# rongzhao-zhang/EfficientQ

Measured on AMD Instinct MI355X. Metric: ptq_calibration_throughput, higher is better.
Workload: dtype i8xi8->i32 (exact) for the Gram systems and per-iteration loss convs of the layers with quantised input, f32/f64 elsewhere

## Files before the change

efficientq_amd/_lib.py:

```python
from __future__ import annotations

import ctypes as C
import os

import torch

_HERE = os.path.dirname(os.path.abspath(__file__))
LIB_PATH = os.path.join(_HERE, "libeffq_hip.so")

EFFQ_OK = 0
_ERR_NAMES = {1: "EFFQ_ERR_ARG", 2: "EFFQ_ERR_HIP", 3: "EFFQ_ERR_WORKSPACE", 4: "EFFQ_ERR_NO_DEVICE",
              5: "EFFQ_ERR_NOT_CONVERGED"}


class EffqError(RuntimeError):
    pass


class Geom(C.Structure):
    _fields_ = [(n, C.c_int32) for n in
                ("N", "C1", "C2", "D", "H", "W", "KD", "KH", "KW", "SD", "SH", "SW", "PD", "PH", "PW")]

    def out_dims(self):
        return ((self.D + 2 * self.PD - self.KD) // self.SD + 1,
# ... 80 lines not shown
    "effq_fp_check": (_I, [_P, _P, _P]),
    "effq_fp_channels_max_row": (_I, []),
    "effq_fixed_point_channels": (_I, [_P, _P, _P, _I, _I, _I, _D, _I, _P, _P, _P, _P]),
    "effq_fixed_point_channels_proj": (_I, [_P, _P, _P, _I, _I, _I, _D, _I, _P, _P, _P, _P, _F, _P, _P, _P, _I, _I, _D,
                                            _D, _P]),
    "effq_gram_packed_elems": (_SZ, [_I, _I]),
    "effq_gram_pack": (_I, [_P, _P, _I, _I, _P, _P]),
    "effq_gram_unpack": (_I, [_P, _I, _I, _P, _P, _P]),
    "effq_act_quant_backward": (_I, [_P, _P, _I, _P, _P, _P, _SZ, _P, _P]),
    "effq_att_classes_ws_bytes": (_SZ, []),
    "effq_att_classes": (_I, [_P, _LL, _P, _P, _P, C.POINTER(C.c_int32), _P, _P]),
    "effq_prof_enable": (_I, [_I]),
    "effq_prof_count": (_I, []),
    "effq_prof_read": (_I, [_I, C.POINTER(ProfRecord)]),
    "effq_admm_num_inverses": (_I, [_D, _D, _I, _I]),
    "effq_admm_run": (_I, [C.POINTER(AdmmRunArgs)]),
    "effq_admm_select_best": (_I, [_P, _I, _P, _P, _SZ, _SZ, _P, _P, _P, _P]),
    "effq_gram_ws_bytes": (_SZ, [_GP, _I]),
    "effq_gram_accum": (_I, [_P, _P, _P, _GP, _I, _P, _P, _I, _P, _SZ, _P]),
    "effq_gram_plan_query": (_I, [_GP, _I, _IP, _IP, _IP, _IP, _LLP, _IP, _IP]),
    "effq_gram_i8_supported": (_I, [_GP, _I]),
    "effq_gram_i8_ws_bytes": (_SZ, [_GP, _I]),
    "effq_gram_accum_i8": (_I, [_P, _P, _GP, _I, _P, _I, _P, _P, _P, _I, _LL, _P, _P, _I, _P, _SZ, _P]),
    "effq_gram_accum_i8_unw": (_I, [_P, _P, _GP, _I, _P, _I, _P, _P, _P, _I, _LL, _P, _P, _I, _P, _P, _P, _SZ, _P]),
    "effq_gram_i8_plan_query": (_I, [_GP, _I, _LL, _IP, _IP, _IP, _IP, _IP, _IP]),
    "effq_gram_i8_group_query": (_I, [_GP, _I, _LL, _IP, _IP, _IP, _IP]),
    "effq_gram_i8_set_group": (_I, [_I, _I]),
    "effq_upsample_trilinear": (_I, [_P, _I, _I, _I, _I, _I, _I, _I, _I, _P, _P]),
    "effq_gram_f64_supported": (_I, [_GP, _I]),
    "effq_gram_f64_ws_bytes": (_SZ, [_GP, _I]),
    "effq_gram_f64": (_I, [_P, _P, _GP, _I, _P, _P, _P, _SZ, _P]),
    "effq_gram_f64_plan_query": (_I, [_GP, _I, _IP, _IP, _IP, _IP]),
    "effq_gram_f64_pipelined": (_I, [_P, _P, _GP, _I]),
    "effq_gram_loss_ws_bytes": (_SZ, [_I]),
    "effq_gram_loss": (_I, [_P, _P, _P, _P, _P, _I, _I, _I, _P, _P, _SZ, _P]),
    "effq_packed_bytes": (_SZ, [_SZ, _I]),
    "effq_pack_levels": (_I, [_P, _SZ, _I, _P, _P]),
    "effq_unpack_levels": (_I, [_P, _SZ, _I, _P, _P]),
    "effq_ainv_ld": (_I, [_I]),
    "effq_fp_bracket_export_words": (_SZ, []),
    "effq_fp_bracket_export": (_I, [_P, _SZ, _P, _P, _SZ, _P]),
    "effq_fp_bracket_rebase": (_I, [_P, _P, _SZ, _P]),
    "effq_fp_bracket_import": (_I, [_P, _SZ, _P, _I, _SZ, _P, _P, _SZ, _P]),
    "effq_admm_uses_traj": (_I, [_SZ, _I]),
    "effq_gram_loss_i8_supported": (_I, [_I, _I, _I, _I]),
    "effq_gram_loss_i8_num_planes": (_I, [C.c_longlong]),
    "effq_gram_loss_i8_planes_bytes": (_SZ, [_I, _I, _I]),
    "effq_gram_loss_i8_prepare": (_I, [_P, _I, _I, _P, _I, _I, _P, _P, _P]),
    "effq_gram_loss_i8_ws_bytes": (_SZ, []),
    "effq_gram_loss_i8": (_I, [_P, _I, _P, _P, _P, _P, _P, _P, _P, _I, _I, _I, _I, _I, _I, _P, _P, _SZ, _P]),
    "effq_spd_inverse_ws_bytes": (_SZ, [_I]),
    "effq_spd_inverse": (_I, [_P, _I, _I, _D, _D, _P, _P, _SZ, _P]),
    "effq_spd_inverse_plan": (_I, [_I, _IP, _IP, _IP]),
    "effq_prox_plan_query": (_I, [_I, _I, _IP, _IP, _IP, _IP]),
    "effq_prox_ws_bytes": (_SZ, [_I, _I]),
    "effq_prox_solve": (_I, [_P, _P, _P, _P, _P, _P, _I, _I, _I, _D, _D, _P, _P, _P, _SZ, _P]),
    "effq_prox_solve_shifted": (_I, [_P, _P, _P, _P, _P, _P, _I, _I, _I, _D, _D, _D, _I, _P, _P, _P, _SZ, _P]),
    "effq_admm_presum": (_I, [_P, _P, _P, _SZ, _P]),
    "effq_admm_project_dual": (_I, [_P, _P, _P, _I, _P, _P, _F, _P, _SZ, _P]),
    "effq_conv_plan_query": (_I, [_GP, _I, _IP, _IP, _IP, _IP, _IP, _IP, _IP, _IP, _LLP]),
    "effq_conv_i8_plan_query": (_I, [_GP, _I, _IP, _IP, _IP, _IP]),
    "effq_conv_i8s_plan_query": (_I, [_GP, _I, _I, _IP, _IP, _IP, _IP, _IP, _IP, _IP]),
    "effq_conv_i8_supported": (_I, [_GP, _I, _I]),
    "effq_conv_i8s_supported": (_I, [_GP, _I, _I]),
    "effq_conv_i8s_ws_bytes": (_SZ, [_GP, _I, _I]),
    "conv3d_calib_step_i8s": (_I, [_P, _P, _P, _P, _GP, _P, _I, _P, _I, _I, _P, _P, _SZ, _P]),
    "effq_conv_i8_ws_bytes": (_SZ, [_GP]),
    "conv3d_calib_step_i8": (_I, [_P, _P, _P, _P, _GP, _P, _I, _P, _I, _P, _P, _SZ, _P]),
    "effq_conv_i8_out_supported": (_I, [_GP, _I, _I]),
    "conv3d_quant_forward_i8": (_I, [_P, _P, _P, _P, _P, _GP, _P, _I, _P, _I, _P, _P, _P, _SZ, _P]),
    "effq_conv_ws_bytes": (_SZ, [_GP]),
    "conv3d_quant_calib_step": (_I, [_P, _P, _P, _P, _P, _GP, _P, _I, _P, _P, _P, _SZ, _P]),
    "effq_adam_step": (_I, [_P, _P, _P, _P, _D, _D, _D, _D, _I, _SZ, _P]),
    "effq_window_gather": (_I, [_P, _I, _I, _I, _I, _I, _I, _I, _I, _I, _I, _I, _I, _I, _I, _P, _P]),
    "effq_window_put": (_I, [_P, _I, _I, _I, _I, _I, _I, _I, _P, _P]),
    "effq_window_stitch": (_I, [_P, _I, _I, _I, _I, _I, _I, _I, _I, _I, _I, _I, _P, _P, _P, _I, _P, _P]),
    "effq_seg_tallies": (_I, [_P, _P, _I, _LL, _I, _I, _F, _P, _P, _SZ, _P]),
    "effq_seg_sweep": (_I, [_P, _P, _I, _LL, _I, _I, _F, _P, _P]),
    "effq_seg_sweep_edges": (_I, [_I, _F, _P]),
    "effq_seg_sweep_plan": (_I, [_I, _LL, _I, _IP, _IP]),
    "effq_seg_labels": (_I, [_P, _I, _I, _LL, _I, _I, _F, _I, _P, _P]),
    "effq_seg_labels_source": (_I, [_P, _I, _P, _P, _P, _P, _P, _I, _I, _F, _P, _P]),
    "effq_seg_probs_source": (_I, [_P, _I, _P, _P, _P, _P, _P, _I, _P, _P, _P]),
    "effq_seg_agreement": (_I, [_P, _P, _I, _LL, _I, _I, _F, _P, _P, _P, _P, _P, _SZ, _P]),
    "effq_cc_ws_bytes": (_SZ, [_I, _I, _I, _I]),
    "effq_cc_label": (_I, [_P, _I, _I, _I, _I, _I, _P, _P, _P, _SZ, _P]),
    "effq_seg_lesions": (_I, [_P, _P, _I, _I, _I, _I, _I, _I, _F, _I, _P, _P, _SZ, _P]),
    "effq_cc_table_ws_bytes": (_SZ, [_I, _I, _I, _I, _I]),
    "effq_cc_table": (_I, [_P, _I, _I, _I, _I, _I, _I, _P, _P, _P, _SZ, _P]),
    "effq_seg_lesion_table": (_I, [_P, _P, _I, _I, _I, _I, _I, _I, _F, _I, _I, _P, _P, _P, _P, _SZ, _P]),
    "effq_label_clean_ws_bytes": (_SZ, [_I, _I, _I]),
    "effq_label_clean": (_I, [_P, _I, _I, _I, _I, _I, _P, _P, _P, _P, _P, _SZ, _P]),
    "effq_label_tallies_ws_bytes": (_SZ, []),
    "effq_label_tallies": (_I, [_P, _P, _I, _I, _LL, _P, _P, _P, _SZ, _P]),
    "effq_surf_ws_bytes": (_SZ, [_I, _I, _I, _I]),
    "effq_edt_sq": (_I, [_P, _I, _I, _I, _I, _P, _P, _SZ, _P]),
    "effq_seg_surface": (_I, [_P, _P, _I, _I, _I, _I, _I, _I, _F, _P, _P, _P, _SZ, _P]),
    "effq_surf_mm_ws_bytes": (_SZ, [_I, _I, _I, _I]),
    "effq_edt_sq_mm": (_I, [_P, _I, _I, _I, _I, _F, _F, _F, _P, _P, _SZ, _P]),
    "effq_seg_surface_mm": (_I, [_P, _P, _I, _I, _I, _I, _I, _I, _F, _F, _F, _F, _P, _P, _P, _P, _SZ, _P]),
    "effq_prep_window": (_I, [_P, _SZ, _F, _F, _P]),
    "effq_prep_resample": (_I, [_P, _I, _I, _I, _I, _D, _D, _D, _I, _P, _I, _I, _I, _P]),
    "effq_prep_bbox_moments": (_I, [_P, _I, _I, _I, _I, _I, _P, _P, _P, _P, _SZ, _P]),
    "effq_prep_sqdev": (_I, [_P, _I, _LL, _I, _P, _P, _P, _SZ, _P]),
    "effq_prep_standardise_crop": (_I, [_P, _I, _I, _I, _I, _I, _P, _P, _P, _P, _P, _P]),
    "effq_prep_crop_u8": (_I, [_P, _I, _I, _I, _I, _P, _P, _P, _P]),
# ... 47 lines not shown
```

efficientq_amd/csrc/solve.hip:

```cpp
#include <cstdlib>
#include <vector>
#include "common.h"
#include "internal.h"

namespace effq {

typedef float f32x16 __attribute__((ext_vector_type(16)));
typedef double f64x4 __attribute__((ext_vector_type(4)));
typedef float f32x4 __attribute__((ext_vector_type(4)));

static inline int round_up(int v, int m) { return (v + m - 1) / m * m; }

constexpr int NBK = 64;
constexpr int LDA_S = 66;
constexpr int LDB_S = 80;

__global__ __launch_bounds__(256) void k_build_a64(const float* __restrict__ A0, int n, int npad, int has_bias,
                                                   double rho, double eta, double* __restrict__ A64) {
  const size_t tot = (size_t)npad * npad;
  const size_t stride = (size_t)gridDim.x * blockDim.x;
  for (size_t e = (size_t)blockIdx.x * blockDim.x + threadIdx.x; e < tot; e += stride) {
    const int i = (int)(e / npad), j = (int)(e % npad);
    double v = 0.0;
    if (i < n && j < n) {
// ... 87 lines not shown
                                                  double* __restrict__ XT) {
  extern __shared__ __attribute__((aligned(16))) double sm[];
  double* As = sm;
  double* Bs = sm + NBK * LDA_S;
  const int kblk = kb / NBK;
  const int t = blockIdx.x;
  const int tid = threadIdx.x, lane = tid & 63, wid = tid >> 6;
  const int wr = wid >> 1, wc = wid & 1;
  if (t == kblk) {
    for (int e = tid; e < NBK * NBK; e += 256) A[(size_t)(kb + (e >> 6)) * npad + kb + (e & 63)] = Dinv[e];
    return;
  }
  const bool upper = t < kblk;
  const double sgn = upper ? -1.0 : 1.0;
  for (int e = tid; e < NBK * NBK; e += 256) {
    const int r = e >> 6, c = e & 63;
    const double v = upper ? A[(size_t)(t * NBK + r) * npad + kb + c] : A[(size_t)(kb + r) * npad + (size_t)t * NBK + c];
    if (upper) {
      As[r * LDA_S + c] = v;
    } else {
      As[c * LDA_S + r] = v;
    }
  }
  load_tile(Bs, LDB_S, Dinv, NBK);
  lds_barrier();
  for (int e = tid; e < NBK * NBK; e += 256) {
    const int kk = e >> 6, r = e & 63;
    XT[(size_t)kk * npad + (size_t)t * NBK + r] = sgn * As[r * LDA_S + kk];
  }
  f64x4 acc[2][2];
#pragma unroll
  for (int mi = 0; mi < 2; ++mi)
#pragma unroll
    for (int ni = 0; ni < 2; ++ni)
#pragma unroll
      for (int r = 0; r < 4; ++r) acc[mi][ni][r] = 0.0;
  tile_mma64(As, Bs, acc);
  const int lr = lane & 15, lk = lane >> 4;
#pragma unroll
  for (int mi = 0; mi < 2; ++mi)
#pragma unroll
    for (int ni = 0; ni < 2; ++ni)
#pragma unroll
      for (int r = 0; r < 4; ++r) {
        const int row = wr * 32 + mi * 16 + lk + 4 * r;
        const int col = wc * 32 + ni * 16 + lr;
        const double z = acc[mi][ni][r];
        NZ[(size_t)(t * NBK + row) * NBK + col] = -z;
        if (upper)
          A[(size_t)(t * NBK + row) * npad + kb + col] = -z;
        else
          A[(size_t)(kb + col) * npad + (size_t)t * NBK + row] = z;
      }
}

__global__ __launch_bounds__(256) void k_gj_trail_sym(double* __restrict__ A, int npad, int kb,
                                                      const double* __restrict__ NZ, const double* __restrict__ XT,
                                                      double* __restrict__ Dinv_next) {
  __shared__ __attribute__((aligned(16))) double As[NBK * LDA_S];
  __shared__ double fcol[2][NBK + 1];
  const int kblk = kb / NBK, nblk = npad / NBK;
  const int kn = kblk + 1;
  const bool ahead = Dinv_next != nullptr && kn < nblk;
  const int tid = threadIdx.x, lane = tid & 63, wid = tid >> 6;
  const int wr = wid >> 1, wc = wid & 1;
  const int lr = lane & 15, lk = lane >> 4;
  if (blockIdx.y == 0) {
    if (blockIdx.x != 0 || !ahead) return;
    for (int e = tid; e < NBK * NBK; e += 256) {
      const int r = e >> 6, c = e & 63;
      As[r * LDA_S + c] = NZ[(size_t)(kn * NBK + r) * NBK + c];
    }
    lds_barrier();
    const double* Cb = A + (size_t)(kn * NBK + wr * 32) * npad + (size_t)kn * NBK + wc * 32;
    const double* Rb = XT + (size_t)kn * NBK + wc * 32;
    f64x4 acc[2][2];
#pragma unroll
    for (int mi = 0; mi < 2; ++mi)
#pragma unroll
      for (int ni = 0; ni < 2; ++ni)
#pragma unroll
        for (int r = 0; r < 4; ++r) acc[mi][ni][r] = Cb[(size_t)(mi * 16 + lk + 4 * r) * npad + ni * 16 + lr];
#pragma unroll 4
    for (int ks = 0; ks < NBK / 4; ++ks) {
      double a[2], b[2];
#pragma unroll
      for (int mi = 0; mi < 2; ++mi) a[mi] = As[(wr * 32 + mi * 16 + lr) * LDA_S + ks * 4 + lk];
#pragma unroll
      for (int ni = 0; ni < 2; ++ni) b[ni] = Rb[(size_t)(ks * 4 + lk) * npad + ni * 16 + lr];
#pragma unroll
      for (int mi = 0; mi < 2; ++mi)
#pragma unroll
        for (int ni = 0; ni < 2; ++ni) acc[mi][ni] = __builtin_amdgcn_mfma_f64_16x16x4f64(a[mi], b[ni], acc[mi][ni], 0, 0, 0);
    }
    lds_barrier();
#pragma unroll
    for (int mi = 0; mi < 2; ++mi)
#pragma unroll
      for (int ni = 0; ni < 2; ++ni)
#pragma unroll
        for (int r = 0; r < 4; ++r)
          As[(wr * 32 + mi * 16 + lk + 4 * r) * LDA_S + wc * 32 + ni * 16 + lr] = acc[mi][ni][r];
    lds_barrier();
    constexpr int CPW = NBK / 4;
    double reg[CPW];
#pragma unroll
    for (int j = 0; j < CPW; ++j) reg[j] = As[lane * LDA_S + wid * CPW + j];
    gj_invert_regs<CPW>(reg, fcol, lane, wid);
#pragma unroll
    for (int j = 0; j < CPW; ++j) Dinv_next[lane * NBK + wid * CPW + j] = reg[j];
    return;
  }
  const int ib = (int)blockIdx.y - 1;
  if (ib == kblk) return;
  if ((int)(blockIdx.x * GJ_CT + GJ_CT - 1) < ib) return;
  for (int e = tid; e < NBK * NBK; e += 256) {
    const int r = e >> 6, c = e & 63;
    As[r * LDA_S + c] = NZ[(size_t)(ib * NBK + r) * NBK + c];
  }
  lds_barrier();
  auto live = [&](int t) -> bool {
    const int jb = blockIdx.x * GJ_CT + t;
    return t < GJ_CT && jb < nblk && jb != kblk && jb >= ib && !(ahead && ib == kn && jb == kn);
  };
  auto fetch = [&](int t, f64x4 (&c)[2][2]) {
    const int jb = blockIdx.x * GJ_CT + t;
    const double* Cb = A + (size_t)(ib * NBK + wr * 32) * npad + (size_t)jb * NBK + wc * 32;
#pragma unroll
    for (int mi = 0; mi < 2; ++mi)
#pragma unroll
      for (int ni = 0; ni < 2; ++ni)
#pragma unroll
        for (int r = 0; r < 4; ++r) c[mi][ni][r] = Cb[(size_t)(mi * 16 + lk + 4 * r) * npad + ni * 16 + lr];
  };
  f64x4 nxt[2][2];
  int t = 0;
  while (t < GJ_CT && !live(t)) ++t;
  if (t < GJ_CT) fetch(t, nxt);
  while (t < GJ_CT) {
    const int jb = blockIdx.x * GJ_CT + t;
    f64x4 acc[2][2];
#pragma unroll
    for (int mi = 0; mi < 2; ++mi)
#pragma unroll
      for (int ni = 0; ni < 2; ++ni) acc[mi][ni] = nxt[mi][ni];
    int tn = t + 1;
    while (tn < GJ_CT && !live(tn)) ++tn;
    if (tn < GJ_CT) fetch(tn, nxt);
    double* Cb = A + (size_t)(ib * NBK + wr * 32) * npad + (size_t)jb * NBK + wc * 32;
    const double* Rb = XT + (size_t)jb * NBK + wc * 32;
#pragma unroll 4
    for (int ks = 0; ks < NBK / 4; ++ks) {
      double a[2], b[2];
#pragma unroll
      for (int mi = 0; mi < 2; ++mi) a[mi] = As[(wr * 32 + mi * 16 + lr) * LDA_S + ks * 4 + lk];
#pragma unroll
      for (int ni = 0; ni < 2; ++ni) b[ni] = Rb[(size_t)(ks * 4 + lk) * npad + ni * 16 + lr];
#pragma unroll
      for (int mi = 0; mi < 2; ++mi)
#pragma unroll
        for (int ni = 0; ni < 2; ++ni) acc[mi][ni] = __builtin_amdgcn_mfma_f64_16x16x4f64(a[mi], b[ni], acc[mi][ni], 0, 0, 0);
    }
#pragma unroll
    for (int mi = 0; mi < 2; ++mi)
#pragma unroll
      for (int ni = 0; ni < 2; ++ni)
#pragma unroll
        for (int r = 0; r < 4; ++r) Cb[(size_t)(mi * 16 + lk + 4 * r) * npad + ni * 16 + lr] = acc[mi][ni][r];
    t = tn;
  }
}

__global__ __launch_bounds__(256) void k_a64_to_f32(const double* __restrict__ A64, int n, int npad,
                                                    float* __restrict__ Ainv, int lda) {
  const size_t tot = (size_t)n * lda;
  const size_t stride = (size_t)gridDim.x * blockDim.x;
  for (size_t e = (size_t)blockIdx.x * blockDim.x + threadIdx.x; e < tot; e += stride) {
    const int i = (int)(e / lda), j = (int)(e % lda);
    const int a = (i < j) ? i : j, b = (i < j) ? j : i;
    Ainv[e] = (j < n) ? (float)A64[(size_t)a * npad + b] : 0.0f;
  }
}

constexpr int WB = 4, WK = WB * NBK;
constexpr int BG_T = 128, BG_KC = 16, BG_LD = 144;
typedef double f64x2 __attribute__((ext_vector_type(2)));

struct GjBig {
  const double* Cin;
  size_t ldin;
  double* Cout;
  size_t ldout;
  int orow, ocol;
  const double* NZT;
  const double* XTW;
  size_t ldx;
  int kdim;
  int nblk;
  int i0m, j0m;
  int skip_lo, skip_hi;
  int la_lo, la_hi;
};

__global__ __launch_bounds__(256, 2) void k_gj_big(const GjBig p) {
  __shared__ __attribute__((aligned(16))) double As[2][BG_KC * BG_LD];
  __shared__ __attribute__((aligned(16))) double Bs[2][BG_KC * BG_LD];
  const int I = p.i0m + (int)blockIdx.y, J = p.j0m + (int)blockIdx.x;
  if (J < I) return;
  auto blk_live = [&](int bi, int bj) -> bool {
    if (bi > bj || bj >= p.nblk) return false;
    if ((bi >= p.skip_lo && bi < p.skip_hi) || (bj >= p.skip_lo && bj < p.skip_hi)) return false;
    if (bi >= p.la_lo && bi < p.la_hi && bj >= p.la_lo && bj < p.la_hi) return false;
    return true;
  };
  if (!(blk_live(2 * I, 2 * J) || blk_live(2 * I, 2 * J + 1) || blk_live(2 * I + 1, 2 * J) || blk_live(2 * I + 1, 2 * J + 1)))
    return;
  const int tid = threadIdx.x, lane = tid & 63, wid = tid >> 6;
  const int wr = wid >> 1, wc = wid & 1;
  const int lr = lane & 15, lk = lane >> 4;
  const int bi = 2 * I + wr, bj = 2 * J + wc;
  const bool live = blk_live(bi, bj);
  f64x4 acc[4][4];
  if (live) {
// ... 653 lines not shown
    int s5 = (256 + tiles5 / 2) / tiles5;
    if (s5 > nkt5 / 16) s5 = nkt5 / 16;
    if (s5 < 1) s5 = 1;
    p.nsplit = s5;
    return p;
  }
  if (p.c2p >= 256) { p.variant = 0; p.gx = (n + 63) / 64; p.gy = p.c2p / 256; }
  else if (p.c2p == 128) { p.variant = 1; p.gx = (n + 63) / 64; p.gy = 1; }
  else if (p.c2p == 64) { p.variant = 2; p.gx = (n + 63) / 64; p.gy = 1; }
  else { p.variant = 3; p.gx = (n + 127) / 128; p.gy = 1; }
  const int tiles = p.gx * p.gy, nkt = p.ldb / PBK;
  int s = (440 + tiles - 1) / tiles;
  if (s > nkt / 6) s = nkt / 6;
  if (s > 16) s = 16;
  if (s < 1) s = 1;
  if (p.variant == 0) {
    const int smax = s > 1 ? 16 : 1;
    double best = -1.0;
    for (int c = 1; c <= smax && c <= nkt / 6; ++c) {
      const int wgs = tiles * c, rounds = (wgs + 767) / 768;
      const double score = (double)wgs / (768.0 * rounds) - 0.01 * c;
      if (score > best) { best = score; s = c; }
    }
  }
  p.nsplit = s;
  return p;
}

}

using namespace effq;

extern "C" {

static size_t gj64_aux_doubles(size_t npad) { return 2 * (size_t)NBK * npad + 2 * NBK * NBK; }

constexpr int GJ_WIDE_MIN_BLOCKS = 100;
static bool gj_takes_wide(int nblk) { return nblk >= GJ_WIDE_MIN_BLOCKS; }
static int gj_wide_pivot(int nblk) { return (nblk >= 100) ? effq::WB : 2; }

size_t effq_spd_inverse_ws_bytes(int n) {
  if (n <= 0) return 0;
  const size_t npad = (size_t)round_up(n, NBK);
  size_t d = npad * npad + gj64_aux_doubles(npad);
  if (gj_takes_wide((int)(npad / NBK))) {
    const size_t ldx = (size_t)round_up((int)npad, BG_T);
    d = npad * npad + 2 * (size_t)WK * ldx + (size_t)WK * WK + gj64_aux_doubles(WK);
  }
  return d * sizeof(double) + 256;
}

int effq_ainv_ld(int n) { return n > 0 ? round_up(n, 32) : 0; }

static int gj64_sweep(double* A64, int npad, double* aux, hipStream_t st) {
  const int nblk = npad / NBK;
  double* XT = aux;
  double* NZ = XT + (size_t)NBK * npad;
  double* Dinv = NZ + (size_t)NBK * npad;
  const size_t lds = (size_t)(NBK * LDA_S + NBK * LDB_S) * sizeof(double);
  for (int k = 0; k < nblk; ++k) {
    const int kb = k * NBK;
    double* Dk = Dinv + (size_t)(k & 1) * NBK * NBK;
    double* Dn = Dinv + (size_t)((k + 1) & 1) * NBK * NBK;
    if (k == 0) hipLaunchKernelGGL(k_gj_diag, dim3(1), dim3(GJD_T), 0, st, A64, npad, kb, Dk);
    hipLaunchKernelGGL(k_gj_panel, dim3(nblk), dim3(256), lds, st, A64, npad, kb, Dk, NZ, XT);
    if (nblk > 1)
      hipLaunchKernelGGL(k_gj_trail_sym, dim3((nblk + GJ_CT - 1) / GJ_CT, nblk + 1), dim3(256), 0, st, A64, npad, kb, NZ,
                         XT, Dn);
    EFFQ_LAUNCH_CHECK();
  }
  return EFFQ_OK;
}

struct GjWideCtx {
  int dev;
  hipStream_t caller, helper;
  hipEvent_t e1, e2;
};
static thread_local std::vector<GjWideCtx> g_gj_ctx;

static int gj_wide_ctx(hipStream_t caller, GjWideCtx** out) {
  int dev = 0;
  EFFQ_HIP(hipGetDevice(&dev));
  for (GjWideCtx& c : g_gj_ctx)
    if (c.dev == dev && c.caller == caller) {
      *out = &c;
      return EFFQ_OK;
    }
  GjWideCtx c;
  c.dev = dev;
  c.caller = caller;
  int prio = 0;
  if (hipStreamGetPriority(caller, &prio) != hipSuccess) prio = 0;
  EFFQ_HIP(hipStreamCreateWithPriority(&c.helper, hipStreamNonBlocking, prio));
  EFFQ_HIP(hipEventCreateWithFlags(&c.e1, hipEventDisableTiming));
  EFFQ_HIP(hipEventCreateWithFlags(&c.e2, hipEventDisableTiming));
  g_gj_ctx.push_back(c);
  *out = &g_gj_ctx.back();
  return EFFQ_OK;
}

static int gj_wide_sweep(double* A64, int npad, double* aux, hipStream_t st) {
  const int nblk = npad / NBK;
  const int WB = gj_wide_pivot(nblk);
  const size_t ldx = (size_t)round_up(npad, BG_T);
  double* NZT = aux;
  double* XTW = NZT + (size_t)WK * ldx;
  double* Dw = XTW + (size_t)WK * ldx;
  double* aux64 = Dw + (size_t)WK * WK;
  const int nK = (nblk + WB - 1) / WB, nm = (nblk + 1) / 2;
  GjWideCtx* ctx = nullptr;
  if (nK > 1) {
    const int rc = gj_wide_ctx(st, &ctx);
    if (rc != EFFQ_OK) return rc;
  }
  hipStream_t s2 = ctx ? ctx->helper : st;
  const size_t lds = (size_t)(NBK * LDA_S + NBK * LDB_S) * sizeof(double);
  const size_t pf_lds = (size_t)(2 * NBK * PF_LD + 2 * (NBK + 1)) * sizeof(double);
  auto pivot_block = [&](int k0, int mk, int kdim, hipStream_t s) -> int {
// ... 33 lines not shown
    }
    hipLaunchKernelGGL(k_gj_wback_w, dim3(nblk, m), dim3(256), 0, s2, A64, npad, kb0, m, Dw, NZT, ldx);
    EFFQ_LAUNCH_CHECK();
    if (mn > 0) {
      const int rc = pivot_block(kn0, mn, m * NBK, s2);
      if (rc != EFFQ_OK) return rc;
    }
    if (nblk > m) {
      GjBig g;
      memset(&g, 0, sizeof(g));
      g.Cin = A64; g.ldin = (size_t)npad;
      g.Cout = A64; g.ldout = (size_t)npad; g.orow = 0; g.ocol = 0;
      g.NZT = NZT; g.XTW = XTW; g.ldx = ldx; g.kdim = m * NBK; g.nblk = nblk;
      g.i0m = 0; g.j0m = 0;
      g.skip_lo = kb0; g.skip_hi = kb0 + m;
      g.la_lo = mn > 0 ? kn0 : -1; g.la_hi = mn > 0 ? kn0 + mn : -1;
      hipLaunchKernelGGL(k_gj_big, dim3(nm, nm), dim3(256), 0, st, g);
      EFFQ_LAUNCH_CHECK();
    }
    if (ctx) {
      EFFQ_HIP(hipEventRecord(ctx->e2, s2));
      EFFQ_HIP(hipStreamWaitEvent(st, ctx->e2, 0));
    }
  }
  return EFFQ_OK;
}

int effq_spd_inverse_prepare(void* stream) {
  GjWideCtx* ctx = nullptr;
  return gj_wide_ctx(as_stream(stream), &ctx);
}

int effq_spd_inverse(const float* A0, int n, int has_bias, double rho, double eta, float* Ainv, void* ws,
                     size_t ws_bytes, void* stream) {
  EFFQ_CHECK_ARG(A0 && Ainv && ws && n > 0);
  EFFQ_CHECK_ARG(eta > 0.0 && rho >= 0.0);
  if (ws_bytes < effq_spd_inverse_ws_bytes(n)) {
    set_error("spd_inverse: workspace %zu < required %zu", ws_bytes, effq_spd_inverse_ws_bytes(n));
    return EFFQ_ERR_WORKSPACE;
  }
  const int npad = round_up(n, NBK);
  double* A64 = reinterpret_cast<double*>(ws);
  double* aux = A64 + (size_t)npad * npad;
  hipStream_t st = as_stream(stream);
  {
    size_t nb = ((size_t)npad * npad + 255) / 256;
    if (nb > 8192) nb = 8192;
    hipLaunchKernelGGL(k_build_a64, dim3((unsigned)nb), dim3(256), 0, st, A0, n, npad, has_bias, rho, eta, A64);
    EFFQ_LAUNCH_CHECK();
  }
  const size_t lds = (size_t)(NBK * LDA_S + NBK * LDB_S) * sizeof(double);
  EFFQ_HIP(raise_lds_limit<k_gj_panel>(lds));
  EFFQ_HIP(raise_lds_limit<k_gj_panel_w>(lds));
  EFFQ_HIP(raise_lds_limit<k_gj_pivot_fused>((2 * NBK * PF_LD + 2 * (NBK + 1)) * sizeof(double)));
  const int rc = gj_takes_wide(npad / NBK) ? gj_wide_sweep(A64, npad, aux, st) : gj64_sweep(A64, npad, aux, st);
  if (rc != EFFQ_OK) return rc;
  {
    const int lda = effq_ainv_ld(n);
    size_t nb = ((size_t)n * lda + 255) / 256;
    if (nb > 8192) nb = 8192;
    hipLaunchKernelGGL(k_a64_to_f32, dim3((unsigned)nb), dim3(256), 0, st, A64, n, npad, Ainv, lda);
    EFFQ_LAUNCH_CHECK();
  }
  return EFFQ_OK;
}

int effq_spd_inverse_plan(int n, int* wide, int* nblk, int* pivot_blocks) {
  EFFQ_CHECK_ARG(n > 0 && wide && nblk && pivot_blocks);
  const int nb = round_up(n, NBK) / NBK;
  *wide = gj_takes_wide(nb) ? 1 : 0;
  *nblk = nb;
  *pivot_blocks = *wide ? (nb + gj_wide_pivot(nb) - 1) / gj_wide_pivot(nb) : nb;
  return EFFQ_OK;
}

int effq_prox_plan_query(int c2, int n, int* variant, int* gx, int* gy, int* nsplit) {
  EFFQ_CHECK_ARG(c2 > 0 && n > 0 && variant && gx && gy && nsplit);
  const ProxPlan p = prox_plan(c2, n);
  *variant = p.variant;
  *gx = p.gx;
  *gy = p.gy;
  *nsplit = p.nsplit;
  return EFFQ_OK;
}

size_t effq_prox_ws_bytes(int c2, int n) {
  if (c2 <= 0 || n <= 0) return 0;
  const ProxPlan p = prox_plan(c2, n);
  return ((size_t)p.c2p + (p.nsplit > 1 ? (size_t)p.nsplit * c2 : 0)) * p.ldb * sizeof(float) + 256;
}

static int prox_solve_impl(const float* B0, const float* Ainv, const float* W0, const float* b0, const float* G,
                           const float* dual, int c2, int n, int has_bias, double rho, double eta, double shift,
                           int nterms, float* wstar, float* bstar, void* ws, size_t ws_bytes, void* stream,
                           bool prebuilt = false, const float** part_out = nullptr, int* nsplit_out = nullptr,
                           int* ldp_out = nullptr) {
  EFFQ_CHECK_ARG(B0 && Ainv && W0 && G && dual && wstar && ws && c2 > 0 && n > 0 && nterms >= 1);
  EFFQ_CHECK_ARG(!has_bias || (b0 != nullptr && bstar != nullptr));
  if (ws_bytes < effq_prox_ws_bytes(c2, n)) {
    set_error("prox_solve: workspace %zu < required %zu", ws_bytes, effq_prox_ws_bytes(c2, n));
    return EFFQ_ERR_WORKSPACE;
  }
  const ProxPlan pl = prox_plan(c2, n);
  const int c2p = pl.c2p, ldb = pl.ldb;
  const int lda = effq_ainv_ld(n);
  float* Bm = reinterpret_cast<float*>(ws);
  float* part = Bm + (size_t)c2p * ldb;
  hipStream_t st = as_stream(stream);
  for (int term = 0; term < nterms; ++term) {
    if (!(prebuilt && term == 0)) {
      const int nw = n - (has_bias ? 1 : 0);
      if ((nw % 4) == 0) {
        const unsigned bx = (unsigned)((ldb / 4 + 255) / 256);
        hipLaunchKernelGGL(k_build_b4, dim3(bx, (unsigned)c2p), dim3(256), 0, st, B0, W0, b0, G, dual, c2, n,
                           has_bias ? 1 : 0, (float)rho, (float)eta, Bm, ldb, (term > 0) ? wstar : nullptr, (float)shift);
      } else {
        size_t nb = ((size_t)c2p * ldb + 255) / 256;
        if (nb > 4096) nb = 4096;
        hipLaunchKernelGGL(k_build_b, dim3((unsigned)nb), dim3(256), 0, st, B0, W0, b0, G, dual, c2, n, has_bias ? 1 : 0,
                           (float)rho, (float)eta, Bm, ldb, c2p, (term > 0) ? wstar : nullptr, (float)shift);
      }
      EFFQ_LAUNCH_CHECK();
    }
    const dim3 grid(pl.gx, pl.gy, pl.nsplit);
#define EFFQ_PROX_LAUNCH(MT, WM, WN, NTN)                                                                              \
  hipLaunchKernelGGL((k_prox_gemm<MT, WM, WN, NTN>), grid, dim3(256), 0, st, Bm, ldb, Ainv, lda, n, c2, has_bias ? 1 : 0, \
                     wstar, bstar, part, ldb)
// ... 79 lines not shown
```

efficientq_amd/hip_ops.py:

```python
from __future__ import annotations

import ctypes as C
import math
from typing import Optional, Tuple

import torch

from . import _lib
from ._lib import Geom, check

ADMM_TOL = 1e-5
FP_BRACKET_MIN = 1 << 18
DP_GATHER_AFTER = 4
DP_GATHER_MAX_BYTES = 128 << 20


def _ptr(t: Optional[torch.Tensor]):
    return None if t is None else C.c_void_p(t.data_ptr())


def to_ndhwc(x: torch.Tensor) -> torch.Tensor:
    return x.permute(0, 2, 3, 4, 1).contiguous()


# ... 534 lines not shown
        check(self.lib.effq_gram_loss_i8(_ptr(planes), int(planes.shape[0]), _ptr(Au), _ptr(Bu), _ptr(syy), _ptr(Gq), _ptr(b),
                                         _ptr(states), _ptr(al), int(act_levels), int(w_levels), c2, n, int(has_b), count,
                                         _ptr(hist), _ptr(ws), ws.numel(), self.stream), "effq_gram_loss_i8")
        return hist

    def gram_reduce(self, A0: torch.Tensor, B0: torch.Tensor, reducer):
        n, c2 = int(A0.shape[0]), int(B0.shape[0])
        buf = torch.empty(self.lib.effq_gram_packed_elems(n, c2), dtype=torch.float32, device=self.device)
        check(self.lib.effq_gram_pack(_ptr(A0), _ptr(B0), n, c2, _ptr(buf), self.stream), "effq_gram_pack")
        reducer(buf)
        check(self.lib.effq_gram_unpack(_ptr(buf), n, c2, _ptr(A0), _ptr(B0), self.stream), "effq_gram_unpack")
        return A0, B0

    @staticmethod
    def storage_bits(levels: int) -> int:
        for b in (1, 2, 4, 8):
            if levels <= (1 << b):
                return b
        raise _lib.EffqError(f"{levels} levels do not fit 8 bits")

    def pack_levels(self, idx: torch.Tensor, bits: int) -> torch.Tensor:
        if idx.dtype != torch.uint8 or not idx.is_contiguous():
            raise _lib.EffqError("pack_levels wants contiguous uint8 level ids")
        nb = self.lib.effq_packed_bytes(idx.numel(), int(bits))
        if idx.numel() and nb == 0:
            raise _lib.EffqError(f"unsupported field width {bits}")
        out = torch.empty(int(nb), dtype=torch.uint8, device=idx.device)
        check(self.lib.effq_pack_levels(_ptr(idx), idx.numel(), int(bits), _ptr(out), self.stream), "effq_pack_levels")
        return out

    def unpack_levels(self, packed: torch.Tensor, n: int, bits: int) -> torch.Tensor:
        if packed.dtype != torch.uint8 or packed.numel() != self.lib.effq_packed_bytes(int(n), int(bits)):
            raise _lib.EffqError("unpack_levels: buffer does not match n and the field width")
        out = torch.empty(int(n), dtype=torch.uint8, device=packed.device)
        check(self.lib.effq_unpack_levels(_ptr(packed.contiguous()), int(n), int(bits), _ptr(out), self.stream),
              "effq_unpack_levels")
        return out

    def spd_inverse(self, A0: torch.Tensor, has_bias: bool, rho: float, eta: float,
                    out: Optional[torch.Tensor] = None, ws_key: str = "inv") -> torch.Tensor:
        n = A0.shape[0]
        A0 = self._f32(A0)
        if out is None:
            out = torch.empty(n, self.lib.effq_ainv_ld(n), dtype=torch.float32, device=self.device)
        ws = self._workspace(ws_key, self.lib.effq_spd_inverse_ws_bytes(n))
        check(self.lib.effq_spd_inverse(_ptr(A0), n, int(has_bias), rho, eta, _ptr(out), _ptr(ws), ws.numel(),
                                        self.stream), "effq_spd_inverse")
        return out

    def spd_inverse_plan(self, n: int) -> dict:
        wide, nblk, piv = C.c_int(), C.c_int(), C.c_int()
        check(self.lib.effq_spd_inverse_plan(int(n), C.byref(wide), C.byref(nblk), C.byref(piv)), "effq_spd_inverse_plan")
        return dict(wide=bool(wide.value), nblk=nblk.value, pivot_blocks=piv.value)

    def prox_plan(self, c2: int, n: int) -> dict:
        v, gx, gy, ns = C.c_int(), C.c_int(), C.c_int(), C.c_int()
        check(self.lib.effq_prox_plan_query(int(c2), int(n), C.byref(v), C.byref(gx), C.byref(gy), C.byref(ns)),
              "effq_prox_plan_query")
        return dict(variant=v.value, gx=gx.value, gy=gy.value, nsplit=ns.value)

    def prox_solve(self, B0, Ainv, W0, b0, G, dual, rho: float, eta: float, wstar, bstar):
        c2, n = B0.shape
        ws = self._workspace("prox", self.lib.effq_prox_ws_bytes(c2, n))
        check(self.lib.effq_prox_solve(_ptr(B0), _ptr(Ainv), _ptr(W0), _ptr(b0), _ptr(G), _ptr(dual), c2, n,
                                       int(b0 is not None), rho, eta, _ptr(wstar), _ptr(bstar), _ptr(ws),
                                       ws.numel(), self.stream), "effq_prox_solve")

    PROX_SHIFT_TERMS = 26

    def prox_solve_shifted(self, B0, Ainv, W0, b0, G, dual, rho: float, eta: float, rho_inv: float, wstar, bstar):
        c2, n = B0.shape
        ws = self._workspace("prox", self.lib.effq_prox_ws_bytes(c2, n))
        terms = self.shift_terms(rho, eta, rho_inv)
        check(self.lib.effq_prox_solve_shifted(_ptr(B0), _ptr(Ainv), _ptr(W0), _ptr(b0), _ptr(G), _ptr(dual), c2, n,
                                               int(b0 is not None), rho, eta, rho_inv, terms, _ptr(wstar),
                                               _ptr(bstar), _ptr(ws), ws.numel(), self.stream),
              "effq_prox_solve_shifted")

    def admm_run(self, A0, B0, W0, b0, geom: Geom, y_ndhwc, *, xq=None, xidx=None, act_alpha=None, act_levels: int = 0,
                 loss_kind: int = 0, rho: float, rho_max: float, eta: float, iters: int, period: int, levels: int,
                 overlap: bool = True, loss_gram=None, residuals: bool = False, channel_wise: bool = False):
        from types import SimpleNamespace
        c2, n = (int(i) for i in B0.shape)
        has_b = b0 is not None
        W0, A0, B0 = self._f32(W0), self._f32(A0), self._f32(B0)
        b0 = self._f32(b0) if has_b else None
        xq = self._f32(xq) if xq is not None else None
        nw = W0.numel()
        y = self._f32(y_ndhwc)
        planes = None
        if loss_gram is not None and len(loss_gram) == 4:
            loss_kind = 5
            planes = loss_gram[3]
            loss_gram = loss_gram[:3]
        elif loss_gram is not None:
            loss_kind = 4
        if channel_wise and loss_kind not in (0, 4):
            raise _lib.EffqError(f"admm_run: channel mode takes loss kinds 0 and 4, not {loss_kind}")
        _check_shapes(geom, xq if loss_kind in (0, 4, 5) else xidx, W0, b0, y)
        if tuple(A0.shape) != (n, n) or nw != c2 * (n - int(has_b)):
            raise _lib.EffqError("admm_run: A0/B0/W0 shapes do not match")
        n_inv = self.lib.effq_admm_num_inverses(float(rho), float(rho_max), int(iters), int(period))
        if n_inv < 1:
            raise _lib.EffqError("admm_run: bad rho schedule")
        dev, f32 = self.device, torch.float32
        ld = self.lib.effq_ainv_ld(n)
# ... 917 lines not shown
```

include/effq_hip.h:

```cpp
#ifndef EFFQ_HIP_H
#define EFFQ_HIP_H

#include <stddef.h>
#include <stdint.h>

#ifdef __cplusplus
extern "C" {
#endif

enum {
  EFFQ_OK = 0,
  EFFQ_ERR_ARG = 1,
  EFFQ_ERR_HIP = 2,
  EFFQ_ERR_WORKSPACE = 3,
  EFFQ_ERR_NO_DEVICE = 4,
  EFFQ_ERR_NOT_CONVERGED = 5
};

typedef struct effq_geom {
  int32_t N, C1, C2;
  int32_t D, H, W;
  int32_t KD, KH, KW;
  int32_t SD, SH, SW;
  int32_t PD, PH, PW;
// ... 86 lines not shown
                    int has_bias, float* A0, float* B0, int accumulate, void* ws, size_t ws_bytes,
                    void* stream);
int effq_gram_plan_query(const effq_geom* g, int has_bias, int* vec, int* nb, int* npairs, int* nsplit,
                         long long* vox_per_split, int* fold, int* finish_blocks);

int effq_gram_i8_supported(const effq_geom* g, int act_levels);
size_t effq_gram_i8_ws_bytes(const effq_geom* g, int ncls);
int effq_gram_accum_i8(const uint8_t* xidx_ndhwc, const float* y_ndhwc, const effq_geom* g, int has_bias,
                       const float* act_alpha_dev, int act_levels, const int32_t* vox_list,
                       const int32_t* chunk_cls, const float* cls_w_dev, int ncls, long long n_list,
                       float* A0, float* B0, int accumulate, void* ws, size_t ws_bytes, void* stream);
int effq_gram_accum_i8_unw(const uint8_t* xidx_ndhwc, const float* y_ndhwc, const effq_geom* g, int has_bias,
                           const float* act_alpha_dev, int act_levels, const int32_t* vox_list, const int32_t* chunk_cls,
                           const float* cls_w_dev, int ncls, long long n_list, float* A0, float* B0, int accumulate,
                           double* Au, double* Bu, void* ws, size_t ws_bytes, void* stream);
int effq_gram_i8_plan_query(const effq_geom* g, int ncls, long long n_list, int* nb, int* nbx, int* npairs, int* nchunks,
                            int* cps, int* nsplit);
int effq_gram_i8_group_query(const effq_geom* g, int ncls, long long n_list, int* gi, int* gj, int* ngroups, int* grid_y);
int effq_gram_i8_set_group(int gi, int gj);

int effq_gram_f64_supported(const effq_geom* g, int has_bias);
size_t effq_gram_f64_ws_bytes(const effq_geom* g, int has_bias);
int effq_gram_f64(const float* x_ndhwc, const float* y_ndhwc, const effq_geom* g, int has_bias, double* Au, double* Bu,
                  void* ws, size_t ws_bytes, void* stream);
int effq_gram_f64_plan_query(const effq_geom* g, int has_bias, int* nchunk, int* grid, int* ntiles, int* tpw);
int effq_gram_f64_pipelined(const float* x_ndhwc, const float* y_ndhwc, const effq_geom* g, int has_bias);

size_t effq_gram_loss_ws_bytes(int n);
int effq_gram_loss(const double* Au, const double* Bu, const double* syy_dev, const float* G, const float* b, int c2, int n,
                   int has_bias, double* sqerr_out, void* ws, size_t ws_bytes, void* stream);

int effq_gram_loss_i8_supported(int c2, int n, int has_bias, int w_levels);
int effq_gram_loss_i8_num_planes(long long kmax);
size_t effq_gram_loss_i8_planes_bytes(int n, int has_bias, int nplanes);
int effq_gram_loss_i8_prepare(const double* Au, int n, int has_bias, const float* act_alpha_dev, int act_levels,
                              int nplanes, int8_t* planes, int32_t* err_flag_dev, void* stream);
size_t effq_gram_loss_i8_ws_bytes(void);
int effq_gram_loss_i8(const int8_t* planes, int nplanes, const double* Au, const double* Bu, const double* syy_dev,
                      const int8_t* Gq, const float* b, const effq_fp_state* states, const float* act_alpha_dev,
                      int act_levels, int w_levels, int c2, int n, int has_bias, int count, double* hist_out, void* ws,
                      size_t ws_bytes, void* stream);


size_t effq_att_classes_ws_bytes(void);
int effq_att_classes(const float* att, long long V, int32_t* vox_list, int32_t* chunk_cls, float* cls_w_dev,
                     int32_t* info_host_out, void* ws, void* stream);

int effq_spd_inverse_prepare(void* stream);
int effq_ainv_ld(int n);
size_t effq_spd_inverse_ws_bytes(int n);
int effq_spd_inverse(const float* A0, int n, int has_bias, double rho, double eta, float* Ainv,
                     void* ws, size_t ws_bytes, void* stream);
int effq_spd_inverse_plan(int n, int* wide, int* nblk, int* pivot_blocks);

size_t effq_prox_ws_bytes(int c2, int n);
int effq_prox_solve(const float* B0, const float* Ainv, const float* W0, const float* b0, const float* G,
                    const float* dual, int c2, int n, int has_bias, double rho, double eta, float* wstar,
                    float* bstar, void* ws, size_t ws_bytes, void* stream);
int effq_prox_plan_query(int c2, int n, int* variant, int* gx, int* gy, int* nsplit);

int effq_prox_solve_shifted(const float* B0, const float* Ainv, const float* W0, const float* b0, const float* G,
                            const float* dual, int c2, int n, int has_bias, double rho, double eta,
                            double rho_inv, int nterms, float* wstar, float* bstar, void* ws, size_t ws_bytes,
                            void* stream);

int effq_admm_presum(const float* wstar, const float* dual, float* v, size_t n, void* stream);
int effq_admm_project_dual(const float* v, const float* wstar, const effq_fp_state* state_dev, int levels,
                           float* G, float* dual, float dual_div, int8_t* Gq_out, size_t n, void* stream);
size_t effq_conv_ws_bytes(const effq_geom* g);
int conv3d_quant_calib_step(const float* xq_ndhwc, const float* G, const float* bias, const float* y_fp,
                            const float* att, const effq_geom* g, const float* act_alpha_dev, int act_levels,
                            double* sqerr_out, float* out, void* ws, size_t ws_bytes, void* stream);
int effq_conv_plan_query(const effq_geom* g, int loss_only, int* kind, int* fast, int* cslab, int* nslab, int* nt,
                         int* grid_x, int* grid_y, int* ntiles, long long* lds_bytes);

int effq_conv_i8_supported(const effq_geom* g, int act_levels, int w_levels);
size_t effq_conv_i8_ws_bytes(const effq_geom* g);
int conv3d_calib_step_i8(const uint8_t* xidx_ndhwc, const int8_t* Gq, const float* bias, const float* y_fp,
                         const effq_geom* g, const float* act_alpha_dev, int act_levels,
                         const effq_fp_state* w_state_dev, int w_levels, double* sqerr_out, void* ws,
                         size_t ws_bytes, void* stream);
int effq_conv_i8_out_supported(const effq_geom* g, int act_levels, int w_levels);
int conv3d_quant_forward_i8(const uint8_t* xidx_ndhwc, const int8_t* Gq, const float* bias, const float* y_fp,
                            const float* att, const effq_geom* g, const float* act_alpha_dev, int act_levels,
                            const effq_fp_state* w_state_dev, int w_levels, double* sqerr_out, float* out, void* ws,
                            size_t ws_bytes, void* stream);
int effq_conv_i8_plan_query(const effq_geom* g, int want_out, int* kernel, int* grid_x, int* grid_y, int* ntiles);

int effq_conv_i8s_supported(const effq_geom* g, int act_levels, int w_levels);
size_t effq_conv_i8s_ws_bytes(const effq_geom* g, int act_levels, int w_levels);
int conv3d_calib_step_i8s(const uint8_t* xidx_ndhwc, const int8_t* Gq, const float* bias, const float* y_fp,
                          const effq_geom* g, const float* act_alpha_dev, int act_levels,
                          const effq_fp_state* w_state_dev, int w_levels, int prepare, double* sqerr_out,
                          void* ws, size_t ws_bytes, void* stream);
int effq_conv_i8s_plan_query(const effq_geom* g, int act_levels, int w_levels, int* nj, int* ct, int* taps, int* k,
                             int* aoff, int* wmul, int* grid);

int effq_act_quant_backward(const float* x, const float* alpha_dev, int levels, const float* gq, float* gx_out,
                            double* galpha_out, size_t n, void* ws, void* stream);
int effq_adam_step(float* p, const float* g, float* m, float* v, double lr, double b1, double b2, double eps,
                   int t, size_t n, void* stream);

typedef struct effq_admm_run_args {
  const float* A0; const float* B0; const float* W0; const float* b0;
  int32_t c2, n, has_bias, w_levels;
  int32_t iters, rho_period;
// ... 152 lines not shown
```

Measured before the change: 25.46.

## Pack four trailing-update row blocks per 1024-thread workgroup in Gauss-Jordan sweep

Adds a trailing-update kernel variant for the blocked Gauss-Jordan SPD inverse. Each 1024-thread workgroup handles four row blocks and uses 1 or 2 column tiles per strip, chosen by block count. The look-ahead diagonal inverse is computed with 16 waves instead of 4. The goal is to cut per-workgroup launch/latency overhead and raise parallelism for mid-sized matrices, at the cost of larger LDS use and a shared barrier across idle row slots. A runtime switch (default on) selects the new path.

```diff
diff --git a/efficientq_amd/_lib.py b/efficientq_amd/_lib.py
--- a/efficientq_amd/_lib.py
+++ b/efficientq_amd/_lib.py
@@ -156,6 +156,8 @@
     "effq_spd_inverse_ws_bytes": (_SZ, [_I]),
     "effq_spd_inverse": (_I, [_P, _I, _I, _D, _D, _P, _P, _SZ, _P]),
     "effq_spd_inverse_plan": (_I, [_I, _IP, _IP, _IP]),
+    "effq_spd_inverse_set_pivot": (_I, [_I]),
+    "effq_spd_inverse_pivot": (_I, []),
     "effq_prox_plan_query": (_I, [_I, _I, _IP, _IP, _IP, _IP]),
     "effq_prox_ws_bytes": (_SZ, [_I, _I]),
     "effq_prox_solve": (_I, [_P, _P, _P, _P, _P, _P, _I, _I, _I, _D, _D, _P, _P, _P, _SZ, _P]),
diff --git a/efficientq_amd/csrc/solve.hip b/efficientq_amd/csrc/solve.hip
--- a/efficientq_amd/csrc/solve.hip
+++ b/efficientq_amd/csrc/solve.hip
@@ -163,6 +163,66 @@
         else
           A[(size_t)(kb + col) * npad + (size_t)t * NBK + row] = z;
       }
+}
+
+template <int CT>
+__device__ __forceinline__ void gj_trail_strip(double* __restrict__ A, int npad, const double* __restrict__ XT,
+                                               const double* As, int ib, int strip, int kblk, int nblk, bool ahead,
+                                               int t4) {
+  const int lane = t4 & 63, wid = t4 >> 6;
+  const int wr = wid >> 1, wc = wid & 1;
+  const int lr = lane & 15, lk = lane >> 4;
+  const int kn = kblk + 1;
+  auto live = [&](int t) -> bool {
+    const int jb = strip * CT + t;
+    return t < CT && jb < nblk && jb != kblk && jb >= ib && !(ahead && ib == kn && jb == kn);
+  };
+  auto fetch = [&](int t, f64x4 (&c)[2][2]) {
+    const int jb = strip * CT + t;
+    const double* Cb = A + (size_t)(ib * NBK + wr * 32) * npad + (size_t)jb * NBK + wc * 32;
+#pragma unroll
+    for (int mi = 0; mi < 2; ++mi)
+#pragma unroll
+      for (int ni = 0; ni < 2; ++ni)
+#pragma unroll
+        for (int r = 0; r < 4; ++r) c[mi][ni][r] = Cb[(size_t)(mi * 16 + lk + 4 * r) * npad + ni * 16 + lr];
+  };
+  f64x4 nxt[2][2];
+  int t = 0;
+  while (t < CT && !live(t)) ++t;
+  if (t < CT) fetch(t, nxt);
+  while (t < CT) {
+    const int jb = strip * CT + t;
+    f64x4 acc[2][2];
+#pragma unroll
+    for (int mi = 0; mi < 2; ++mi)
+#pragma unroll
+      for (int ni = 0; ni < 2; ++ni) acc[mi][ni] = nxt[mi][ni];
+    int tn = t + 1;
+    while (tn < CT && !live(tn)) ++tn;
+    if (tn < CT) fetch(tn, nxt);
+    double* Cb = A + (size_t)(ib * NBK + wr * 32) * npad + (size_t)jb * NBK + wc * 32;
+    const double* Rb = XT + (size_t)jb * NBK + wc * 32;
+#pragma unroll 4
+    for (int ks = 0; ks < NBK / 4; ++ks) {
+      double a[2], b[2];
+#pragma unroll
+      for (int mi = 0; mi < 2; ++mi) a[mi] = As[(wr * 32 + mi * 16 + lr) * LDA_S + ks * 4 + lk];
+#pragma unroll
+      for (int ni = 0; ni < 2; ++ni) b[ni] = Rb[(size_t)(ks * 4 + lk) * npad + ni * 16 + lr];
+#pragma unroll
+      for (int mi = 0; mi < 2; ++mi)
+#pragma unroll
+        for (int ni = 0; ni < 2; ++ni) acc[mi][ni] = __builtin_amdgcn_mfma_f64_16x16x4f64(a[mi], b[ni], acc[mi][ni], 0, 0, 0);
+    }
+#pragma unroll
+    for (int mi = 0; mi < 2; ++mi)
+#pragma unroll
+      for (int ni = 0; ni < 2; ++ni)
+#pragma unroll
+        for (int r = 0; r < 4; ++r) Cb[(size_t)(mi * 16 + lk + 4 * r) * npad + ni * 16 + lr] = acc[mi][ni][r];
+    t = tn;
+  }
 }
 
 __global__ __launch_bounds__(256) void k_gj_trail_sym(double* __restrict__ A, int npad, int kb,
@@ -230,56 +290,73 @@
     As[r * LDA_S + c] = NZ[(size_t)(ib * NBK + r) * NBK + c];
   }
   lds_barrier();
-  auto live = [&](int t) -> bool {
-    const int jb = blockIdx.x * GJ_CT + t;
-    return t < GJ_CT && jb < nblk && jb != kblk && jb >= ib && !(ahead && ib == kn && jb == kn);
-  };
-  auto fetch = [&](int t, f64x4 (&c)[2][2]) {
-    const int jb = blockIdx.x * GJ_CT + t;
-    const double* Cb = A + (size_t)(ib * NBK + wr * 32) * npad + (size_t)jb * NBK + wc * 32;
-#pragma unroll
-    for (int mi = 0; mi < 2; ++mi)
-#pragma unroll
-      for (int ni = 0; ni < 2; ++ni)
-#pragma unroll
-        for (int r = 0; r < 4; ++r) c[mi][ni][r] = Cb[(size_t)(mi * 16 + lk + 4 * r) * npad + ni * 16 + lr];
-  };
-  f64x4 nxt[2][2];
-  int t = 0;
-  while (t < GJ_CT && !live(t)) ++t;
-  if (t < GJ_CT) fetch(t, nxt);
-  while (t < GJ_CT) {
-    const int jb = blockIdx.x * GJ_CT + t;
-    f64x4 acc[2][2];
-#pragma unroll
-    for (int mi = 0; mi < 2; ++mi)
-#pragma unroll
-      for (int ni = 0; ni < 2; ++ni) acc[mi][ni] = nxt[mi][ni];
-    int tn = t + 1;
-    while (tn < GJ_CT && !live(tn)) ++tn;
-    if (tn < GJ_CT) fetch(tn, nxt);
-    double* Cb = A + (size_t)(ib * NBK + wr * 32) * npad + (size_t)jb * NBK + wc * 32;
-    const double* Rb = XT + (size_t)jb * NBK + wc * 32;
-#pragma unroll 4
+  gj_trail_strip<GJ_CT>(A, npad, XT, As, ib, (int)blockIdx.x, kblk, nblk, ahead, tid);
+}
+
+constexpr int GJT_Q = 4;
+constexpr size_t GJT16_LDS = (size_t)(GJT_Q * NBK * LDA_S + 2 * (NBK + 1)) * sizeof(double);
+template <int CT>
+__global__ __launch_bounds__(256 * GJT_Q) void k_gj_trail_sym16(double* __restrict__ A, int npad, int kb,
+                                                               const double* __restrict__ NZ,
+                                                               const double* __restrict__ XT,
+                                                               double* __restrict__ Dinv_next) {
+  extern __shared__ __attribute__((aligned(16))) double sm[];
+  double(*fcol)[NBK + 1] = reinterpret_cast<double(*)[NBK + 1]>(sm + GJT_Q * NBK * LDA_S);
+  const int kblk = kb / NBK, nblk = npad / NBK;
+  const int kn = kblk + 1;
+  const bool ahead = Dinv_next != nullptr && kn < nblk;
+  const int tid = threadIdx.x, lane = tid & 63, wid = tid >> 6;
+  if (blockIdx.y == 0) {
+    if (blockIdx.x != 0 || !ahead) return;
+    double* As = sm;
+    double* Ms = sm + NBK * LDA_S;
+    const int tr = wid >> 2, tc = wid & 3;
+    const int lr = lane & 15, lk = lane >> 4;
+    const double* Cb = A + (size_t)(kn * NBK + tr * 16) * npad + (size_t)kn * NBK + tc * 16;
+    const double* Rb = XT + (size_t)kn * NBK + tc * 16;
+    constexpr int ZPT = NBK * NBK / (256 * GJT_Q);
+    double z[ZPT], b[NBK / 4];
+    f64x4 acc;
+#pragma unroll
+    for (int i = 0; i < ZPT; ++i) z[i] = NZ[(size_t)kn * NBK * NBK + i * 256 * GJT_Q + tid];
+#pragma unroll
+    for (int r = 0; r < 4; ++r) acc[r] = Cb[(size_t)(lk + 4 * r) * npad + lr];
+#pragma unroll
+    for (int ks = 0; ks < NBK / 4; ++ks) b[ks] = Rb[(size_t)(ks * 4 + lk) * npad + lr];
+#pragma unroll
+    for (int i = 0; i < ZPT; ++i) {
+      const int e = i * 256 * GJT_Q + tid;
+      As[(e >> 6) * LDA_S + (e & 63)] = z[i];
+    }
+    lds_barrier();
+#pragma unroll
     for (int ks = 0; ks < NBK / 4; ++ks) {
-      double a[2], b[2];
-#pragma unroll
-      for (int mi = 0; mi < 2; ++mi) a[mi] = As[(wr * 32 + mi * 16 + lr) * LDA_S + ks * 4 + lk];
-#pragma unroll
-      for (int ni = 0; ni < 2; ++ni) b[ni] = Rb[(size_t)(ks * 4 + lk) * npad + ni * 16 + lr];
-#pragma unroll
-      for (int mi = 0; mi < 2; ++mi)
-#pragma unroll
-        for (int ni = 0; ni < 2; ++ni) acc[mi][ni] = __builtin_amdgcn_mfma_f64_16x16x4f64(a[mi], b[ni], acc[mi][ni], 0, 0, 0);
-    }
-#pragma unroll
-    for (int mi = 0; mi < 2; ++mi)
-#pragma unroll
-      for (int ni = 0; ni < 2; ++ni)
-#pragma unroll
-        for (int r = 0; r < 4; ++r) Cb[(size_t)(mi * 16 + lk + 4 * r) * npad + ni * 16 + lr] = acc[mi][ni][r];
-    t = tn;
-  }
+      const double a = As[(tr * 16 + lr) * LDA_S + ks * 4 + lk];
+      acc = __builtin_amdgcn_mfma_f64_16x16x4f64(a, b[ks], acc, 0, 0, 0);
+    }
+#pragma unroll
+    for (int r = 0; r < 4; ++r) Ms[(tr * 16 + lk + 4 * r) * LDA_S + tc * 16 + lr] = acc[r];
+    lds_barrier();
+    constexpr int CPW = NBK / (4 * GJT_Q);
+    double reg[CPW];
+#pragma unroll
+    for (int j = 0; j < CPW; ++j) reg[j] = Ms[lane * LDA_S + wid * CPW + j];
+    gj_invert_regs<CPW>(reg, fcol, lane, wid);
+#pragma unroll
+    for (int j = 0; j < CPW; ++j) Dinv_next[lane * NBK + wid * CPW + j] = reg[j];
+    return;
+  }
+  const int q = wid >> 2, t4 = tid & 255;
+  const int ib = ((int)blockIdx.y - 1) * GJT_Q + q;
+  const bool work = ib < nblk && ib != kblk && (int)(blockIdx.x * CT + CT - 1) >= ib;
+  double* As = sm + q * NBK * LDA_S;
+  if (work)
+    for (int e = t4; e < NBK * NBK; e += 256) {
+      const int r = e >> 6, c = e & 63;
+      As[r * LDA_S + c] = NZ[(size_t)(ib * NBK + r) * NBK + c];
+    }
+  lds_barrier();
+  if (work) gj_trail_strip<CT>(A, npad, XT, As, ib, (int)blockIdx.x, kblk, nblk, ahead, t4);
 }
 
 __global__ __launch_bounds__(256) void k_a64_to_f32(const double* __restrict__ A64, int n, int npad,
@@ -1039,8 +1116,14 @@
 
 int effq_ainv_ld(int n) { return n > 0 ? round_up(n, 32) : 0; }
 
+static int g_gj_pivot = 1;
+
+constexpr int GJ_T16_ONE_MAX = 47, GJ_T16_TWO_MAX = 55;
+static int gj_trail16_strip(int nblk) { return nblk <= GJ_T16_ONE_MAX ? 1 : nblk <= GJ_T16_TWO_MAX ? 2 : 0; }
+
 static int gj64_sweep(double* A64, int npad, double* aux, hipStream_t st) {
   const int nblk = npad / NBK;
+  const int ct16 = g_gj_pivot != 0 ? gj_trail16_strip(nblk) : 0;
   double* XT = aux;
   double* NZ = XT + (size_t)NBK * npad;
   double* Dinv = NZ + (size_t)NBK * npad;
@@ -1051,7 +1134,12 @@
     double* Dn = Dinv + (size_t)((k + 1) & 1) * NBK * NBK;
     if (k == 0) hipLaunchKernelGGL(k_gj_diag, dim3(1), dim3(GJD_T), 0, st, A64, npad, kb, Dk);
     hipLaunchKernelGGL(k_gj_panel, dim3(nblk), dim3(256), lds, st, A64, npad, kb, Dk, NZ, XT);
-    if (nblk > 1)
+    const dim3 rows16((nblk + GJT_Q - 1) / GJT_Q + 1), wg16(256 * GJT_Q);
+    if (nblk > 1 && ct16 == 1)
+      hipLaunchKernelGGL(k_gj_trail_sym16<1>, dim3(nblk, rows16.x), wg16, GJT16_LDS, st, A64, npad, kb, NZ, XT, Dn);
+    else if (nblk > 1 && ct16 == 2)
+      hipLaunchKernelGGL(k_gj_trail_sym16<2>, dim3((nblk + 1) / 2, rows16.x), wg16, GJT16_LDS, st, A64, npad, kb, NZ, XT, Dn);
+    else if (nblk > 1)
       hipLaunchKernelGGL(k_gj_trail_sym, dim3((nblk + GJ_CT - 1) / GJ_CT, nblk + 1), dim3(256), 0, st, A64, npad, kb, NZ,
                          XT, Dn);
     EFFQ_LAUNCH_CHECK();
@@ -1191,6 +1279,8 @@
   const size_t lds = (size_t)(NBK * LDA_S + NBK * LDB_S) * sizeof(double);
   EFFQ_HIP(raise_lds_limit<k_gj_panel>(lds));
   EFFQ_HIP(raise_lds_limit<k_gj_panel_w>(lds));
+  EFFQ_HIP(raise_lds_limit<k_gj_trail_sym16<1>>(GJT16_LDS));
+  EFFQ_HIP(raise_lds_limit<k_gj_trail_sym16<2>>(GJT16_LDS));
   EFFQ_HIP(raise_lds_limit<k_gj_pivot_fused>((2 * NBK * PF_LD + 2 * (NBK + 1)) * sizeof(double)));
   const int rc = gj_takes_wide(npad / NBK) ? gj_wide_sweep(A64, npad, aux, st) : gj64_sweep(A64, npad, aux, st);
   if (rc != EFFQ_OK) return rc;
@@ -1212,6 +1302,14 @@
   *pivot_blocks = *wide ? (nb + gj_wide_pivot(nb) - 1) / gj_wide_pivot(nb) : nb;
   return EFFQ_OK;
 }
+
+int effq_spd_inverse_set_pivot(int variant) {
+  EFFQ_CHECK_ARG(variant == 0 || variant == 1);
+  g_gj_pivot = variant;
+  return EFFQ_OK;
+}
+
+int effq_spd_inverse_pivot(void) { return g_gj_pivot; }
 
 int effq_prox_plan_query(int c2, int n, int* variant, int* gx, int* gy, int* nsplit) {
   EFFQ_CHECK_ARG(c2 > 0 && n > 0 && variant && gx && gy && nsplit);
diff --git a/efficientq_amd/hip_ops.py b/efficientq_amd/hip_ops.py
--- a/efficientq_amd/hip_ops.py
+++ b/efficientq_amd/hip_ops.py
@@ -610,6 +610,9 @@
         wide, nblk, piv = C.c_int(), C.c_int(), C.c_int()
         check(self.lib.effq_spd_inverse_plan(int(n), C.byref(wide), C.byref(nblk), C.byref(piv)), "effq_spd_inverse_plan")
         return dict(wide=bool(wide.value), nblk=nblk.value, pivot_blocks=piv.value)
+
+    def spd_inverse_set_pivot(self, variant: int) -> None:
+        check(self.lib.effq_spd_inverse_set_pivot(int(variant)), "effq_spd_inverse_set_pivot")
 
     def prox_plan(self, c2: int, n: int) -> dict:
         v, gx, gy, ns = C.c_int(), C.c_int(), C.c_int(), C.c_int()
diff --git a/include/effq_hip.h b/include/effq_hip.h
--- a/include/effq_hip.h
+++ b/include/effq_hip.h
@@ -162,6 +162,8 @@
 int effq_spd_inverse(const float* A0, int n, int has_bias, double rho, double eta, float* Ainv,
                      void* ws, size_t ws_bytes, void* stream);
 int effq_spd_inverse_plan(int n, int* wide, int* nblk, int* pivot_blocks);
+int effq_spd_inverse_set_pivot(int variant);
+int effq_spd_inverse_pivot(void);
 
 size_t effq_prox_ws_bytes(int c2, int n);
 int effq_prox_solve(const float* B0, const float* Ainv, const float* W0, const float* b0, const float* G,
```

After: 25.39. No clear change (-0.3%).
